# gradientpm/gvpm

Measured on AMD Instinct MI355X. Metric: photon gather+shift evaluations per second (G-BRE 3D), higher is better.
Workload: dtype f32; 1 GPU; BASELINE configs[1]: S-cbox + homogeneous medium, G-BRE 3D kernel, 512x512 frame, 1000000 photons/iter, 227 SPPM iters, initialScaleVolume 1.0; technique=bre3d, scene=cbox, photons_per_iter=1000000

## Files before the change

gvpm_amd/csrc/context.h:

```cpp
#pragma once
#include <dlfcn.h>
#include <hip/hip_runtime.h>
#include <rccl/rccl.h>

#include <cmath>
#include <cstdio>
#include <cstdlib>
#include <cstring>
#include <algorithm>
#include <chrono>
#include <string>
#include <vector>

#include "device_types.h"
#include "scene_bvh.h"

namespace gvpm {
hipError_t sortPairsU32(SortTemp &tmp, const uint32_t *kIn, uint32_t *kOut, const uint32_t *vIn, uint32_t *vOut,
                        uint32_t n, int endBit, hipStream_t s);
void launch_bounds(const float *pos, uint32_t n, float *partial, int nblocks, float *out6, float *hostOut,
                   hipStream_t s, const uint32_t *word = nullptr, uint32_t *wordOut = nullptr);
hipError_t reserveScanTemp(SortTemp &tmp, uint32_t n);
void launch_bundle_fit(const gvpm_camera_ray *rays, uint32_t nsets, int pass, const Grid &g, double *out, hipStream_t s);
void launch_export_u32(const uint32_t *a, const uint32_t *b, const uint32_t *c, const uint32_t *d, const uint32_t *e, uint32_t *hostOut,
// ... 19 lines not shown
void launch_tile_start(const uint32_t *start, uint32_t ntiles, uint32_t shift, uint32_t *tileStart, hipStream_t s);
void launch_segment_start(const uint32_t *keys, uint32_t n, uint32_t nseg, uint32_t shift, uint32_t *start,
                          hipStream_t s);
void launch_beam_keys(const gvpm_camera_ray *rays, uint32_t nsets, int width, int tw, int th, uint32_t *keys,
                      uint32_t *vals, hipStream_t s);
void launch_plan_bre(const GatherArgs &a, int beamsPerWave, uint32_t ntiles, uint32_t target, uint4 *items,
                     uint32_t *itemCount, uint2 *itemOff, uint32_t *blockTotal, uint32_t itemCap, hipStream_t stream);
uint32_t eval_unit_pairs();
void launch_traverse_bre(const GatherArgs &a, int beamsPerWave, const uint4 *items, const uint2 *itemOff,
                         const uint32_t *itemCount, uint32_t *queueHead, uint32_t *pairs, uint32_t *pairCnt,
                         uint32_t nwaves, bool persistent, hipStream_t stream, uint2 *units = nullptr, uint32_t *unitCtl = nullptr,
                         uint32_t unitCap = 0);
void launch_apply_host_shifts_beams(const GatherArgs &a, const gvpm_host_shift *results, uint32_t n, hipStream_t s);
void launch_evaluate_primal(const GatherArgs &a, int beamsPerWave, const uint4 *items, const uint2 *itemOff,
                            const uint32_t *itemCount, uint32_t *queueHead, const uint32_t *pairs, const uint32_t *pairCnt,
                            uint32_t nwaves, hipStream_t stream);
void launch_evaluate_bre(const GatherArgs &a, int beamsPerWave, bool fullVis, const uint4 *items, const uint2 *itemOff,
                         const uint32_t *itemCount, uint32_t *queueHead, const uint32_t *pairs, const uint32_t *pairCnt,
                         uint32_t nwaves, bool persistent, hipStream_t stream, const uint2 *units = nullptr,
                         const uint32_t *unitCtl = nullptr, uint32_t unitCap = 0);
uint32_t plan_items_capacity(uint32_t nsets, uint32_t ntiles, int beamsPerWave);
void launch_build_chain(ChainArgs c, const GatherArgs &a, const gvpm_photon_soa &raw, int beamsPerWave, uint32_t target, uint4 *items,
                        uint2 *itemOff, uint32_t itemCap, float dmax, const NearGrid &ng, uint32_t extCap, uint32_t *origIdx,
                        uint32_t *hostOut, bool initBuckets, hipStream_t s, uint32_t pairCapBlocks = 0xFFFFFFFFu, uint32_t unitCap = 0,
                        uint32_t unitPairs = 1, bool fullVis = false);
struct PoissonGraphCache {
  hipGraph_t graph = nullptr;
  hipGraphExec_t exec = nullptr;
  void *scratch = nullptr;
  int W = 0, H = 0, cgMax = 0;
  float alpha = 0.f;
};
void poisson_graph_release(PoissonGraphCache &c);
hipError_t poisson_solve_device(const gvpm_poisson_params &prm, int W, int H, const float *dx, const float *dy,
                                const float *tp, const float *direct, float *out, void *scratch,
                                PoissonGraphCache &cache, hipStream_t s);
size_t poisson_scratch_bytes(int W, int H);
void launch_finalize(float *accum, const float *iter, size_t n, int it, uint64_t nbPaths, hipStream_t s);
void launch_scale(const float *in, float *out, size_t n, float scale, hipStream_t s);
void launch_film(const float *acc, const float *emission, int w, int h, int it, int reusePrimal, float invDiv,
                 float *thr, float *dx, float *dy, hipStream_t s);
void launch_gather_vpm(const GatherArgs &a, bool fullVis, bool primal, hipStream_t stream);
void launch_vpm_find(const GatherArgs &a, const VpmSplit &sp, hipStream_t stream);
void launch_vpm_redo(const GatherArgs &a, const VpmSplit &sp, bool fullVis, uint32_t nwaves, hipStream_t stream);
void launch_vpm_eval(const GatherArgs &a, const VpmSplit &sp, bool fullVis, uint32_t wavesPerShard, hipStream_t stream);
void launch_vpm_finish(float *accum, float *iter, float *scaleVol, float *nVol, float *mvol, size_t n, float alpha,
                       uint32_t *maxScaleBits, hipStream_t stream);
void launch_accumulate(float *accum, float *iter, size_t n, uint32_t *zeroWord, hipStream_t stream);
// ... 127 lines not shown
  }
  void release() {
    hot.release(); cold.release(); overflowCtr.release(); origIdx.release(); cellStart.release(); cellCount.release(); cellSub.release(); sat.release();
    beamCount.release(); beamStart.release(); keysA.release(); keysB.release();
    valsA.release(); valsB.release(); boundsPartial.release(); bounds6.release(); bKeysA.release(); bKeysB.release();
    bValsA.release(); setPerm.release(); tileStart.release(); items.release(); itemOff.release(); planBoxes.release(); queueCtl.release();
    if (sortTmp.d) (void)hipFree(sortTmp.d);
    sortTmp.d = nullptr;
    sortTmp.bytes = 0;
    pairs.release(); pairCnt.release(); nearExt.release(); chainBuckets.release(); units.release(); notes.release(); notesCount.release();
    if (lastUse) (void)hipEventDestroy(lastUse);
    if (traversed) (void)hipEventDestroy(traversed);
    lastUse = traversed = nullptr;
  }
};

struct gvpm_context {
  int device = 0;
  hipStream_t stream = nullptr;
  hipStream_t streamB = nullptr;
  hipStream_t bstream = nullptr;
  hipStream_t streamC = nullptr;
  hipStream_t streamA2 = nullptr;
  bool evalAlt = false;
  int evalToggle = 0;
  hipEvent_t exactDone = nullptr;
  bool exactDoneValid = false;
  hipStream_t lastEvalStream = nullptr;
  bool travStream = true;
  BuildSet sets[3];
  BuildSet *bs = &sets[0];
  int setIdx = 0;
  bool travOnBuild = true;
  bool beamsExact = false;
  bool bundleEnabled = false;
  bool bundleFromEnv = false;
  bool bundleAuto = false;
  int bundleState = 0, bundleViolations = 0;
  int lastGridMode = 0;
  uint32_t lastGridCells = 0;
  float bundleDiv = 2.f;
  Grid bundleGrid{};
  bool buildChain = true;
  DevBuf<uint32_t> chainCtl;
  bool planBoxHandOff = true;
  bool beamsFreeCone = true;
// ... 209 lines not shown
```

gvpm_amd/csrc/gather_bre.hip:

```cpp
#include <hip/hip_runtime.h>

#include <cstdlib>
#include <type_traits>

#include "device_types.h"
#include "shift_device.h"
#include "tile_walk.h"
#include "vec.h"

namespace gvpm {

struct HitGeom {
  double disk, distSqr;
};

__device__ __forceinline__ HitGeom hitGeom(f3 pf, f3 of, f3 df) {
#pragma clang fp contract(off)
  const double px = pf.x, py = pf.y, pz = pf.z;
  const double ox = of.x, oy = of.y, oz = of.z;
  const double dx = df.x, dy = df.y, dz = df.z;
  const double cx = px - ox, cy = py - oy, cz = pz - oz;
  HitGeom g;
  g.disk = cx * dx + cy * dy + cz * dz;
  const double qx = ox + dx * g.disk, qy = oy + dy * g.disk, qz = oz + dz * g.disk;
// ... 400 lines not shown
  sf = sflux * ws;
  wb = bc * w;
}

template <int B, typename LDS> __device__ __forceinline__ void flushAcc(LDS &s, Acc27 &acc, uint32_t beam) {
#pragma unroll
  for (int k = 0; k < 27; ++k) {
    atomicAdd(&s.acc[k][beam], (double)(acc.v[k]));
    acc.v[k] = 0.f;
  }
}

__device__ __forceinline__ void waveLdsSync() {
  __builtin_amdgcn_fence(__ATOMIC_RELEASE, "wavefront");
  __builtin_amdgcn_wave_barrier();
  __builtin_amdgcn_fence(__ATOMIC_ACQUIRE, "wavefront");
}

#ifndef GVPM_TRAV_WPB
#define GVPM_TRAV_WPB 1
#endif
constexpr int TRAV_WPB = GVPM_TRAV_WPB;
#ifndef GVPM_TRAV_MINW
#define GVPM_TRAV_MINW 5
#endif
#ifndef GVPM_TRAV_OWN_MINW
#define GVPM_TRAV_OWN_MINW 4
#endif
#ifndef GVPM_EVAL_UNIT
#define GVPM_EVAL_UNIT 1280
#endif
#ifndef GVPM_EVAL_UNIT_SMALL
#define GVPM_EVAL_UNIT_SMALL 256
#endif
constexpr uint32_t EVAL_UNIT = GVPM_EVAL_UNIT, EVAL_UNIT_SMALL = GVPM_EVAL_UNIT_SMALL;
struct alignas(16) TravLds {
  float x[STAGE], y[STAGE], z[STAGE];
  uint32_t bits[STAGE];
  uint32_t stageIdx[STAGE];
  float4 cyl[3];
};
typedef float v2f __attribute__((ext_vector_type(2)));

template <int B, bool OWN_WALK>
__global__ __launch_bounds__(64 * TRAV_WPB) __attribute__((amdgpu_waves_per_eu(OWN_WALK ? GVPM_TRAV_OWN_MINW : GVPM_TRAV_MINW))) void traverse_bre_kernel(GatherArgs a, const uint4 *__restrict__ items,
                                                          const uint2 *__restrict__ itemOff,
                                                          const uint32_t *__restrict__ itemCount, uint32_t *queueHead,
// ... 202 lines not shown
                total += t;
              }
              if (B == 16) {
                const uint32_t t = (uint32_t)__shfl_xor((int)c, 16, 64);
                const uint32_t pairSum = c + t;
                const uint32_t t2 = (uint32_t)__shfl_xor((int)pairSum, 32, 64);
                before = ((lane & 16) ? t : 0u) + ((lane & 32) ? t2 : 0u);
                total = pairSum + t2;
              }
              uint32_t off = mine + before;
              while (cm) {
                const uint32_t u = (uint32_t)__ffs(cm) - 1u;
                cm &= cm - 1u;
                if (off < cap) outBase[outOff + off] = s.stageIdx[j0 + u];
                else nOver++;
                ++off;
              }
              mine += total;
            }
          }
        }
      }
    }
    if (sub == 0) pairCnt[(size_t)it * B + b] = (uint32_t)b < nb ? min(mine, cap) : 0u;
    if (units) {
      uint32_t tot = (sub == 0 && (uint32_t)b < nb) ? min(mine, cap) : 0u;
#pragma unroll
      for (int o = 32; o > 0; o >>= 1) tot += (uint32_t)__shfl_xor((int)tot, o, 64);
      tot = (uint32_t)__builtin_amdgcn_readfirstlane((int)tot);
      if (tot) {
        const uint32_t parts = (tot + EVAL_UNIT - 1u) / EVAL_UNIT;
        const uint32_t cls = (tot + parts - 1u) / parts > EVAL_UNIT_SMALL ? 0u : 1u;
        uint32_t slot = 0;
        if (lane == 0) slot = atomicAdd(&unitCtl[cls], parts);
        slot = (uint32_t)__builtin_amdgcn_readfirstlane((int)slot);
        for (uint32_t pp = (uint32_t)lane; pp < parts; pp += 64u) {
          if (slot + pp < unitCap) units[(size_t)cls * unitCap + slot + pp] = make_uint2(it, pp | (parts << 16));
          else nOver++;
        }
      }
    }
    nCand += tested * nb;
  }
  {
#pragma unroll
    for (int o = 32; o > 0; o >>= 1) nOver += (uint32_t)__shfl_xor((int)nOver, o, 64);
    if (lane == 0 && (nCand | nOver)) {
      unsigned long long *row = statRow(a);
      atomicAdd(&row[1], nCand);
      if (nOver) atomicAdd(&row[7], (unsigned long long)nOver);
    }
  }
}

#ifndef GVPM_EVAL_MINW
#define GVPM_EVAL_MINW 3
#endif
#ifndef GVPM_EVAL_ATTR
#define GVPM_EVAL_ATTR
#endif
// ... 567 lines not shown
```

gvpm_amd/csrc/gather_drivers.hip:

```cpp
#include "context.h"

float currentRadius(const gvpm_context *h) {
  return h->cfg.bsphere_radius * h->globalScaleVolume * 0.01f;
}

static int ilog2ceil(uint32_t v) {
  int b = 0;
  while ((1ull << b) < v) ++b;
  return b;
}

struct ChainPrep {
  bool on = false;
  float dmax = 0.f;
  bool wantOrig = false;
  uint32_t *sub = nullptr;
  uint32_t nkeys = 0, tileShift = 0;
  int tw = 4, th = 4;
};
static void beamTiling(const gvpm_context *h, int beamsPerWave, int &tw, int &th, uint32_t &ntiles, int &tileShift) {
  tw = 8;
  th = 4;
  if (beamsPerWave == 64) th = 8;
  if (beamsPerWave == 16) tw = 4;
// ... 658 lines not shown
    c.width = h->cfg.width;
    c.tw = cp.tw;
    c.th = cp.th;
    c.tileShift = cp.tileShift;
    c.ntiles = h->bs->ntiles;
    c.bKeys = h->bs->bKeysA.p;
    c.bRank = h->bs->bValsA.p;
    c.setPerm = h->bs->setPerm.p;
    c.tileStart = h->bs->tileStart.p;
    c.blockSum = reinterpret_cast<uint32_t *>(h->bs->sortTmp.d);
    c.ctl = h->chainCtl.p;
    c.queueCtl = h->bs->queueCtl.p;
    c.overflowCtr = h->bs->overflowCtr.p;
    c.nearExt = h->bs->nearExt.p;
    c.sat = h->bs->sat.p;
    h->boundsPending = h->haveCachedBounds;
    const bool optimistic = h->optimistic && h->pipeline && attempt == 0 && !primal && h->persistentEval && h->lastItems > 0 &&
                            h->bs->pairs.cap >= 128u && h->bs->pairCnt.cap >= (size_t)itemCap * h->beamsPerWave &&
                            (!h->evalUnits || h->bs->units.cap >= 2u);
    const bool fullVisOpt = !h->cfg.visibility_as_written || prevOverflow;
    const bool refuse = optimistic && h->optRefuseEvery > 0 && (++h->optSteps % h->optRefuseEvery) == 0;
    launch_build_chain(c, a, h->rawDev, h->beamsPerWave, h->planTarget, h->bs->items.p, h->bs->itemOff.p, itemCap, cp.dmax, h->nearGrid,
                       (uint32_t)std::min<size_t>(h->bs->nearExt.cap, 0xFFFFFF00u), cp.wantOrig ? h->bs->origIdx.p : nullptr, h->pinCtl,
                       !h->bs->bucketsInit, h->bstream,
                       optimistic ? (refuse ? 0u : (uint32_t)std::min<size_t>((h->bs->pairs.cap - 64u) / 64u, 0xFFFFFFF0u)) : 0xFFFFFFFFu,
                       optimistic && h->evalUnits ? (uint32_t)std::min<size_t>(h->bs->units.cap / 2u, 0x3FFFFFFFu) : 0u, eval_unit_pairs(),
                       fullVisOpt);
    h->bs->bucketsInit = true;
    chainRan = true;
    if (optimistic) {
      HIP_TRY(h, hipEventRecord(evBuild->second, h->bstream));
      const uint32_t guess = std::min<uint32_t>(itemCap, h->lastItems + h->lastItems / 8u + 256u);
      rc = queueGather(0u, guess, true, fullVisOpt);
      if (rc != GVPM_OK) {
        h->bstream = h->stream;
        return rc;
      }
      queued = true;
    }
  } else {
    HIP_TRY(h, hipMemsetAsync(h->bs->queueCtl.p, 0, 8 * sizeof(uint32_t), h->bstream));
    launch_plan_bre(a, h->beamsPerWave, h->bs->ntiles, h->planTarget, h->bs->items.p, h->bs->queueCtl.p, h->bs->itemOff.p,
                    h->bs->queueCtl.p + 3, itemCap, h->bstream);
    launch_export_u32(h->bs->queueCtl.p + 3, rebuilt ? h->bs->overflowCtr.p : nullptr, rebuilt ? h->bs->nearExt.p : nullptr,
                      h->bs->queueCtl.p, h->bs->queueCtl.p + 4, h->pinCtl, h->bstream);
  }
  if (!queued) HIP_TRY(h, hipEventRecord(evBuild->second, h->bstream));
  lap("plan");
  HIP_TRY(h, hipStreamSynchronize(h->bstream));
  lap("syncB");
  blocks = h->pinCtl[0];
  nItems = h->pinCtl[3];
  if (queued && h->pinCtl[5] != 0u) {
    if (getenv("GVPM_TRACE_PLAN")) fprintf(stderr, "[plan] optimistic step refused by the build (status %u): queued again\n", h->pinCtl[5]);
    HIP_TRY(h, hipStreamSynchronize(h->stream));
    if (h->pipeline && h->travStream) HIP_TRY(h, hipStreamSynchronize(h->streamC));
    HIP_TRY(h, hipMemsetAsync(h->bs->queueCtl.p + 1, 0, 2 * sizeof(uint32_t), h->bstream));
    HIP_TRY(h, hipMemsetAsync(h->bs->queueCtl.p + 5, 0, 3 * sizeof(uint32_t), h->bstream));
    HIP_TRY(h, hipStreamSynchronize(h->bstream));
    queued = false;
    h->optRefused++;
  }
  if (a.grid.mode == 1 && h->pinCtl[4] != 0u && attempt == 0) {
    h->bundleState = ++h->bundleViolations > 3 ? -1 : 0;
    h->photonsDirty = true;
    h->boundsPending = false;
    force3D = true;
    continue;
  }
  break;
  }
  h->lastGridMode = a.grid.mode;
  h->lastGridCells = a.grid.ncells;
  if (nItems > itemCap) {
    h->bstream = h->stream;
    return fail(h, GVPM_ERR_STATE, "G-BRE planner produced more work items than its bound");
  }
  if (getenv("GVPM_TRACE_PLAN")) {
    uint32_t q[4] = {0, 0, 0, 0};
// ... 704 lines not shown
```

gvpm_amd/csrc/grid_build.hip:

```cpp
#include <hip/hip_runtime.h>
#include <hipcub/hipcub.hpp>

#include "bundle_grid.h"
#include "device_types.h"
#include "shift_device.h"
#include "tile_walk.h"
#include "vec.h"

namespace gvpm {

__global__ __launch_bounds__(256) void bounds_kernel(const float *__restrict__ pos, uint32_t n, float *partial) {
  __shared__ float red[6][4];
  float mn[3] = {INFINITY, INFINITY, INFINITY}, mx[3] = {-INFINITY, -INFINITY, -INFINITY};
  for (uint32_t i = blockIdx.x * blockDim.x + threadIdx.x; i < n; i += gridDim.x * blockDim.x) {
#pragma unroll
    for (int c = 0; c < 3; ++c) {
      const float v = pos[3 * (size_t)i + c];
      mn[c] = fminf(mn[c], v);
      mx[c] = fmaxf(mx[c], v);
    }
  }
  const int wave = threadIdx.x / 64, lane = threadIdx.x % 64;
#pragma unroll
  for (int c = 0; c < 3; ++c) {
// ... 1112 lines not shown
  const uint32_t base = starts[c.beamOff];
  if (b < nSatBlocks + nBeamBlocks) {
    const uint32_t i = (b - nSatBlocks) * 256u + threadIdx.x;
    if (i < c.nsets) {
      const size_t k = (size_t)c.beamOff + c.bKeys[i];
      c.setPerm[starts[k] - base + (atomicSub(&c.counts[k], 1u) - 1u)] = i;
    }
    return;
  }
  const uint32_t t = (b - nSatBlocks - nBeamBlocks) * 256u + threadIdx.x;
  if (t <= c.ntiles) c.tileStart[t] = starts[(size_t)c.beamOff + ((size_t)t << c.tileShift)] - base;
}

struct TailArgs {
  uint32_t ntiles, target, itemCap, nPlan;
  uint4 *items;
  uint2 *itemOff;
  uint32_t *itemCount, *blockTotal;
  RawPhotons raw;
  const uint32_t *keys, *rank, *cellStart, *sub;
  uint32_t *counts;
  uint32_t *subCount;
  uint32_t n, ncells, extCap;
  uint32_t every;
  float dmax;
  NearGrid ng;
  uint32_t *nearExt, *overflow, *origIdx;
  float4 *hot, *cold;
  uint32_t *ctl;
  const uint32_t *bundleFlag;
  uint32_t *hostOut;
  uint32_t pairCapBlocks;
  uint32_t unitCap, unitPairs;
  uint32_t fullVis;
  uint32_t planGroups;
};
constexpr uint32_t TAIL_PLAN_STAGE = 128;
template <int B> constexpr size_t tailLdsBytes() {
  constexpr size_t pl = sizeof(PlanLds<B, TAIL_PLAN_STAGE>) > sizeof(PlanLdsQ<B, TAIL_PLAN_STAGE>) ? sizeof(PlanLds<B, TAIL_PLAN_STAGE>)
                                                                                                  : sizeof(PlanLdsQ<B, TAIL_PLAN_STAGE>);
  return pl > sizeof(ReorderLds) ? pl : sizeof(ReorderLds);
}
#ifndef GVPM_TAIL_WPE
#define GVPM_TAIL_WPE 6
#endif
template <int B, int MODE> __global__ __launch_bounds__(64) __attribute__((amdgpu_waves_per_eu(GVPM_TAIL_WPE, GVPM_TAIL_WPE))) void chain_tail_kernel(GatherArgs a, TailArgs t) {
  __shared__ __attribute__((aligned(16))) unsigned char ldsRaw[tailLdsBytes<B>()];
  const uint32_t b = blockIdx.x, pslot = b / t.every;
  if (b % t.every == 0u && pslot < t.nPlan) {
    if (a.grid.mode != 1 && t.planGroups)
      planBodyQ<B, TAIL_PLAN_STAGE>(a, t.ntiles, t.target, t.items, t.itemCount, t.itemOff, t.blockTotal, t.itemCap, pslot, t.nPlan,
                                    *reinterpret_cast<PlanLdsQ<B, TAIL_PLAN_STAGE> *>(ldsRaw));
    else
      planBody<B, TAIL_PLAN_STAGE>(a, t.ntiles, t.target, t.items, t.itemCount, t.itemOff, t.blockTotal, t.itemCap, pslot, t.nPlan,
                                   *reinterpret_cast<PlanLds<B, TAIL_PLAN_STAGE> *>(ldsRaw));
  }
  else
    reorderBody<MODE>(t.raw, t.keys, t.rank, t.cellStart, t.n, a.cfg, a.bvh, a.tri4, a.ntri, t.dmax, t.ng, t.nearExt, t.extCap, t.hot,
                      t.cold, t.overflow, t.origIdx, t.sub, t.ncells, b - min(t.nPlan, (b + t.every - 1u) / t.every), t.counts,
                      t.subCount, *reinterpret_cast<ReorderLds *>(ldsRaw));
  if (!lastBlockArrives(t.ctl, blockIdx.x, gridDim.x)) return;
  if (threadIdx.x == 0) {
    t.hostOut[0] = coherentRead(t.blockTotal);
    t.hostOut[1] = coherentRead(t.overflow);
    t.hostOut[2] = coherentRead(t.nearExt);
    t.hostOut[3] = coherentRead(t.itemCount);
    t.hostOut[4] = t.bundleFlag ? coherentRead(const_cast<uint32_t *>(t.bundleFlag)) : 0u;
    uint32_t bad = 0u;
    if (t.pairCapBlocks != 0xFFFFFFFFu) {
      const uint32_t blocks = t.hostOut[0], nIt = t.hostOut[3];
      if (blocks > t.pairCapBlocks) bad |= 1u;
      if (nIt > t.itemCap) bad |= 2u;
      if (t.unitCap && (unsigned long long)blocks * 64ull / t.unitPairs + nIt + 64ull > (unsigned long long)t.unitCap) bad |= 4u;
      if (t.hostOut[1] != 0u && !t.fullVis) bad |= 8u;
      if (t.hostOut[4] != 0u) bad |= 16u;
    }
    t.itemCount[7] = bad;
    t.hostOut[5] = bad;
    __threadfence_system();
  }
}

template <int B>
static void launchTail(int mode, uint32_t grid, hipStream_t s, const GatherArgs &a, const TailArgs &t) {
  if (mode == 0) hipLaunchKernelGGL((chain_tail_kernel<B, 0>), dim3(grid), dim3(64), 0, s, a, t);
  else if (mode == 2) hipLaunchKernelGGL((chain_tail_kernel<B, 2>), dim3(grid), dim3(64), 0, s, a, t);
  else hipLaunchKernelGGL((chain_tail_kernel<B, 1>), dim3(grid), dim3(64), 0, s, a, t);
}

void launch_build_chain(ChainArgs c, const GatherArgs &a, const gvpm_photon_soa &raw, int beamsPerWave, uint32_t target, uint4 *items,
                        uint2 *itemOff, uint32_t itemCap, float dmax, const NearGrid &ng, uint32_t extCap, uint32_t *origIdx,
                        uint32_t *hostOut, bool initBuckets, hipStream_t s, uint32_t pairCapBlocks, uint32_t unitCap, uint32_t unitPairs,
                        bool fullVis) {
  c.nPhBlocks = (c.n + 255u) / 256u;
  c.nBeamBlocks = (c.nsets + 255u) / 256u;
  if (initBuckets) hipLaunchKernelGGL(chain_init_buckets_kernel, dim3(1), dim3(768), 0, s, c.buckets);
  hipLaunchKernelGGL(chain_count_kernel, dim3(c.nPhBlocks + c.nBeamBlocks), dim3(256), 0, s, c);
  if (c.g.mode == 1)
    hipLaunchKernelGGL(chain_stripes_kernel, dim3((c.g.ncells + 255) / 256), dim3(256), 0, s, c.sub, c.sub + (size_t)CELL_STRIPES * c.g.ncells,
                       c.g.ncells, c.counts);
  const uint32_t nScan = (c.scanLen + SCAN_TILE - 1) / SCAN_TILE;
  hipLaunchKernelGGL(chain_scan_reduce_kernel, dim3(nScan), dim3(SCAN_BLOCK), 0, s, c);
  hipLaunchKernelGGL(chain_scan_down_kernel, dim3(nScan), dim3(SCAN_BLOCK), 0, s, c);
  const uint32_t nx1 = c.g.dim[0] + 1, ny1 = c.g.dim[1] + 1;
  const uint32_t nSat = (nx1 * (uint32_t)c.g.dim[2] + 255u) / 256u, nTile = (c.ntiles + 1u + 255u) / 256u;
  hipLaunchKernelGGL(chain_mid_kernel, dim3(nSat + c.nBeamBlocks + nTile), dim3(256), 0, s, c, nSat, c.nBeamBlocks);
  hipLaunchKernelGGL(sat_z_kernel, dim3((nx1 * ny1 + 255) / 256), dim3(256), 0, s, c.g, c.sat);
  TailArgs t{};
  t.ntiles = c.ntiles;
  t.target = target;
  t.itemCap = itemCap;
  t.planGroups = getenv("GVPM_PLAN_GROUPS") ? (atoi(getenv("GVPM_PLAN_GROUPS")) != 0) : 1u;
  {
    const uint32_t per = (t.planGroups && c.g.mode != 1) ? (uint32_t)(64 / (beamsPerWave > 0 ? beamsPerWave : 16)) : 1u;
    const uint32_t want = (c.ntiles + per - 1u) / per;
    t.nPlan = want < 4093u ? std::max(1u, want) : 4093u;
// ... 9 lines not shown
  t.rank = c.rank;
  t.cellStart = c.starts;
  t.sub = c.g.mode == 1 ? c.sub + (size_t)CELL_STRIPES * c.g.ncells : nullptr;
  t.subCount = c.g.mode == 1 ? c.sub : nullptr;
  t.counts = c.g.mode == 1 ? nullptr : c.counts;
  t.n = c.n;
  t.ncells = c.g.ncells;
  t.extCap = extCap;
  t.dmax = dmax;
  t.ng = ng;
  t.nearExt = c.nearExt;
  t.overflow = c.overflowCtr;
  t.origIdx = origIdx;
  t.hot = const_cast<float4 *>(a.hot);
  t.cold = const_cast<float4 *>(a.cold);
  t.ctl = c.ctl + 65;
  t.bundleFlag = a.bundleFlag;
  t.hostOut = hostOut;
  t.pairCapBlocks = pairCapBlocks;
  t.unitCap = unitCap;
  t.unitPairs = unitPairs ? unitPairs : 1u;
  t.fullVis = fullVis ? 1u : 0u;
  const int mode = a.ntri <= 64u ? 0 : (ng.start ? 2 : 1);
  const uint32_t grid = t.nPlan + (c.n + 63u) / 64u;
  t.every = std::max(1u, grid / std::max(1u, t.nPlan));
  switch (beamsPerWave) {
    case 64: launchTail<64>(mode, grid, s, a, t); break;
    case 32: launchTail<32>(mode, grid, s, a, t); break;
    default: launchTail<16>(mode, grid, s, a, t); break;
  }
}

}
```

gvpm_amd/csrc/gvpm_api.hip:

```cpp
#include "context.h"

RcclApi g_rccl;

static const char *validateParams(const gvpm_params *p) {
  if (p->abi_version != GVPM_ABI_VERSION) return "abi_version mismatch";
  if (p->width <= 0 || p->height <= 0 || p->width > 65535 || p->height > 65535) return "bad film size";
  if (p->vol_technique < GVPM_VOL_BRE2D || p->vol_technique > GVPM_VOL_PLANE0D) return "unknown vol_technique";
  const bool use3D = p->vol_technique == GVPM_DISTANCE || p->vol_technique == GVPM_VOL_BRE3D ||
                     (p->vol_technique >= GVPM_BEAM_BEAM_3D_NAIVE && p->vol_technique <= GVPM_BEAM_BEAM_3D_OPTIMIZED);
  if (p->use_shift_null && !use3D && p->vol_technique != GVPM_BEAM_BEAM_1D)
    return "Not possible to shift null without using 3D kernel";
  if (p->max_depth <= 1 && p->max_depth != -1 && p->max_depth != 0) return "Maximum depth must be set to \"2\" or higher!";
  if (!(p->bsphere_radius > 0.f)) return "bsphere_radius must be positive";
  if (!(p->epsilon > 0.f) || !(p->shadow_epsilon > 0.f)) return "epsilon / shadow_epsilon must be positive";
  if (!std::isfinite(p->alpha) || !(p->alpha > 0.f) || p->alpha > 1.f) return "alpha must be in (0, 1]";
  if (p->vol_technique == GVPM_VOL_PLANE0D && p->min_depth < 2) return "Impossible to use plane with minDepth smaller than 2";
  if (!p->no_medium_shift) return "noMediumShift=false is not supported (shiftPhotonMedium is SAssert(false))";
  return nullptr;
}

extern "C" {

int gvpm_abi_version(void) { return GVPM_ABI_VERSION; }

// ... 5 lines not shown
  if (validateParams(params)) {
    const char *m = validateParams(params);
    return (strstr(m, "shift null") || strstr(m, "noMediumShift")) ? GVPM_ERR_UNSUPPORTED : GVPM_ERR_INVALID_ARG;
  }
  int ndev = 0;
  if (hipGetDeviceCount(&ndev) != hipSuccess || ndev <= 0 || device < 0 || device >= ndev) return GVPM_ERR_NO_DEVICE;
  if (hipSetDevice(device) != hipSuccess) return GVPM_ERR_NO_DEVICE;
  gvpm_context *h = new gvpm_context();
  h->device = device;
  h->cfg = *params;
  int prA = 0, prB = 1, prC = -1;
  {
    int least = 0, greatest = 0;
    if (hipDeviceGetStreamPriorityRange(&least, &greatest) == hipSuccess) {
      prB = std::min(prB, least);
      prC = std::max(prC, greatest);
    }
  }
  if (const char *e = getenv("GVPM_STREAM_PRIORITIES")) (void)sscanf(e, "%d,%d,%d", &prA, &prB, &prC);
  if (hipStreamCreateWithPriority(&h->stream, hipStreamNonBlocking, prA) != hipSuccess ||
      hipStreamCreateWithPriority(&h->streamB, hipStreamNonBlocking, prB) != hipSuccess ||
      hipStreamCreateWithPriority(&h->streamC, hipStreamNonBlocking, prC) != hipSuccess ||
      hipStreamCreateWithPriority(&h->streamA2, hipStreamNonBlocking, prA) != hipSuccess ||
      hipEventCreateWithFlags(&h->sets[0].lastUse, hipEventDisableTiming) != hipSuccess ||
      hipEventCreateWithFlags(&h->sets[1].lastUse, hipEventDisableTiming) != hipSuccess ||
      hipEventCreateWithFlags(&h->sets[2].lastUse, hipEventDisableTiming) != hipSuccess ||
      hipEventCreateWithFlags(&h->sets[0].traversed, hipEventDisableTiming) != hipSuccess ||
      hipEventCreateWithFlags(&h->sets[1].traversed, hipEventDisableTiming) != hipSuccess ||
      hipEventCreateWithFlags(&h->sets[2].traversed, hipEventDisableTiming) != hipSuccess) {
    gvpm_destroy(h);
    return GVPM_ERR_HIP;
  }
  if (hipStreamCreateWithFlags(&h->copyStream, hipStreamNonBlocking) != hipSuccess) {
    gvpm_destroy(h);
    return GVPM_ERR_HIP;
  }
  for (int k = 0; k < 3; ++k)
    if (hipEventCreateWithFlags(&h->phSlot[k].copied, hipEventDisableTiming) != hipSuccess ||
        hipEventCreateWithFlags(&h->phSlot[k].consumed, hipEventDisableTiming) != hipSuccess ||
        hipEventCreateWithFlags(&h->phSlot[k].consumedB, hipEventDisableTiming) != hipSuccess ||
        hipEventCreateWithFlags(&h->raySlot[k].copied, hipEventDisableTiming) != hipSuccess ||
        hipEventCreateWithFlags(&h->raySlot[k].freed, hipEventDisableTiming) != hipSuccess) {
      gvpm_destroy(h);
      return GVPM_ERR_HIP;
    }
  h->bstream = h->stream;
// ... 32 lines not shown
  if (const char *e = getenv("GVPM_TRAV_WAVES_PER_CU")) {
    int v = atoi(e);
    if (v >= 1 && v <= 32) h->nwavesTrav = h->ncu * (uint32_t)v;
  }
  {
    if (h->nwavesTrav > GVPM_STAT_ROWS) h->nwavesTrav = GVPM_STAT_ROWS;
    if (h->nwaves > GVPM_STAT_ROWS) h->nwaves = GVPM_STAT_ROWS;
  }
  if (const char *e = getenv("GVPM_PIPELINE")) h->pipeline = atoi(e) != 0;
  if (!h->pipeline && !getenv("GVPM_WAVES_PER_CU") && h->ncu) h->nwaves = std::min<uint32_t>(h->ncu * 12u, GVPM_STAT_ROWS);
  if (const char *e = getenv("GVPM_PERSISTENT")) h->persistentEval = (atoi(e) & 1) != 0, h->persistentTrav = (atoi(e) & 2) != 0;
  if (const char *e = getenv("GVPM_TRAV_ON_BUILD")) h->travOnBuild = atoi(e) != 0;
  if (const char *e = getenv("GVPM_NEAR_GRID")) h->useNearGrid = atoi(e) != 0;
  if (const char *e = getenv("GVPM_TRAV_STREAM")) h->travStream = atoi(e) != 0;
  if (const char *e = getenv("GVPM_BEAMS_FP64")) h->beamsExact = atoi(e) != 0;
  if (const char *e = getenv("GVPM_BEAMS_FREE_CONE")) h->beamsFreeCone = atoi(e) != 0;
  if (const char *e = getenv("GVPM_PLAN_BOXES")) h->planBoxHandOff = atoi(e) != 0;
  if (const char *e = getenv("GVPM_BUILD_CHAIN")) h->buildChain = atoi(e) != 0;
  if (const char *e = getenv("GVPM_EVAL_UNITS")) h->evalUnits = atoi(e) != 0;
  if (const char *e = getenv("GVPM_OPTIMISTIC")) h->optimistic = atoi(e) != 0;
  if (const char *e = getenv("GVPM_OPTIMISTIC_REFUSE")) h->optRefuseEvery = (uint32_t)std::max(0, atoi(e));
  if (const char *e = getenv("GVPM_CLIP_GRID")) h->clipGrid = atoi(e) != 0;
  if (const char *e = getenv("GVPM_EVAL_ALT")) h->evalAlt = atoi(e) != 0;
  if (const char *e = getenv("GVPM_VPM_ORDER")) h->vpmNoOrder = atoi(e) == 0;
  if (const char *e = getenv("GVPM_VPM_SPLIT")) h->vpmSplit = atoi(e) != 0;
  if (const char *e = getenv("GVPM_VPM_PIPELINE")) h->vpmPipeline = atoi(e) != 0;
  if (const char *e = getenv("GVPM_VPM_POOL")) h->vpmPoolPerBatch = (uint32_t)std::max(0, atoi(e));
  if (const char *e = getenv("GVPM_VPM_EVAL_WAVES")) h->vpmEvalWaves = (uint32_t)std::max(64, atoi(e));
  if (const char *e = getenv("GVPM_VPM_REDO_WAVES")) h->vpmRedoWaves = (uint32_t)std::max(1, atoi(e));
  if (const char *e = getenv("GVPM_BEAMS_SPLIT")) h->beamsSplit = atoi(e) != 0;
  if (const char *e = getenv("GVPM_BUNDLE_AUTO")) h->bundleAuto = atoi(e) != 0;
  if (const char *e = getenv("GVPM_BUNDLE")) {
    h->bundleEnabled = atoi(e) != 0;
    h->bundleFromEnv = true;
  }
  if (const char *e = getenv("GVPM_BUNDLE_DIV")) {
    const float v = (float)atof(e);
    if (v >= 0.25f && v <= 16.f) h->bundleDiv = v;
  }
  if (const char *e = getenv("GVPM_BEAM_PAIRS_INIT")) {
    const long long v = atoll(e);
    if (v >= 64 && v <= ((long long)1 << 31)) h->beamPairsInit = (size_t)v;
  }
  if (const char *e = getenv("GVPM_BEAM_ITEMS_INIT")) {
    const long long v = atoll(e);
    if (v >= 1 && v <= ((long long)1 << 30)) h->beamItemsInit = (uint32_t)v;
// ... 20 lines not shown
  }
  *out = h;
  int rc = gvpm_reset(h);
  if (rc != GVPM_OK) {
    gvpm_destroy(h);
    *out = nullptr;
  }
  return rc;
}

int gvpm_destroy(gvpm_context *h) {
  if (!h) return GVPM_ERR_INVALID_ARG;
  (void)hipSetDevice(h->device);
  if (h->stream) (void)hipStreamSynchronize(h->stream);
  if (h->comm && g_rccl.commDestroy) g_rccl.commDestroy(h->comm);
  for (auto &v : h->events)
    for (auto &e : v) {
      (void)hipEventDestroy(e.first);
      (void)hipEventDestroy(e.second);
    }
  if (h->streamB) (void)hipStreamSynchronize(h->streamB);
  if (h->streamC) (void)hipStreamSynchronize(h->streamC);
  if (h->streamA2) (void)hipStreamSynchronize(h->streamA2);
  for (BuildSet &b : h->sets) b.release();
  h->tri4.release(); h->bvh.release();
  for (auto &ps : h->phSlot) {
    ps.raw.release();
    ps.packed.release();
    if (ps.unpacked) (void)hipEventDestroy(ps.unpacked);
    if (ps.copied) (void)hipEventDestroy(ps.copied);
    if (ps.consumed) (void)hipEventDestroy(ps.consumed);
    if (ps.consumedB) (void)hipEventDestroy(ps.consumedB);
  }
  for (auto &rs : h->raySlot) {
    rs.rays.release();
    rs.packed.release();
    if (rs.unpacked) (void)hipEventDestroy(rs.unpacked);
    if (rs.copied) (void)hipEventDestroy(rs.copied);
    if (rs.freed) (void)hipEventDestroy(rs.freed);
  }
  if (h->copyStream) (void)hipStreamDestroy(h->copyStream);
  h->materials.release();
  h->reqHost.release(); h->reqCtx.release(); h->reqCount.release(); h->reqResults.release();
  h->endNOwned.release(); h->subCounts.release(); h->subOffsets.release();
  h->beamCtl.release(); h->beamAux.release(); h->beamClear.release();
  h->nearGridStart.release(); h->nearGridTris.release(); h->nearGridCount.release();
  h->w1Owned.release(); h->len1Owned.release(); h->planeTest.release(); h->beamPairs.release(); h->subFlags.release(); h->shiftExtent.release();
  h->blockKeyA.release(); h->blockKeyB.release(); h->blockValA.release(); h->blockValB.release();
  h->samplesOwned.release(); h->scaleVol.release(); h->nVol.release(); h->mvol.release(); h->maxScaleBits.release();
  poisson_graph_release(h->poissonGraph);
  h->accumTmp.release();
  h->chainCtl.release();
  h->poissonScratch.release(); h->poissonIO.release();
  h->accum.release(); h->accumAll.release(); h->iter.release(); h->filmOut.release(); h->emission.release(); h->stats.release();
  h->exPay.release(); h->exPayCount.release(); h->exOvf.release(); h->exOvfCount.release(); h->exTotals.release();
  if (h->pinB6) (void)hipHostFree(h->pinB6);
  if (h->pinExact) (void)hipHostFree(h->pinExact);
  if (h->pinBeams) (void)hipHostFree(h->pinBeams);
  h->splitId.release(); h->splitMeta.release(); h->splitBlkCnt.release(); h->splitCtl.release(); h->splitK.release();
  h->splitU.release(); h->splitRuns.release();
  if (h->stream) (void)hipStreamDestroy(h->stream);
  if (h->streamB) (void)hipStreamDestroy(h->streamB);
  if (h->streamC) (void)hipStreamDestroy(h->streamC);
  if (h->streamA2) (void)hipStreamDestroy(h->streamA2);
  if (h->exactDone) (void)hipEventDestroy(h->exactDone);
  h->vpmPairs.release(); h->vpmChunkMeta.release(); h->vpmCtl.release(); h->vpmStatus.release(); h->vpmRedo.release(); h->vpmState.release();
  if (h->vpmFound) (void)hipEventDestroy(h->vpmFound);
  if (h->vpmRedone) (void)hipEventDestroy(h->vpmRedone);
  delete h;
  return GVPM_OK;
}

int gvpm_reset(gvpm_context *h) {
  CHECK_H(h);
  {
    const int rcj = joinEvalStreams(h);
    if (rcj != GVPM_OK) return rcj;
  }
  h->reqOutstanding = false;
  h->reqBeams = false;
  if (h->reqCount.p) HIP_TRY(h, hipMemsetAsync(h->reqCount.p, 0, 8, h->stream));
  h->vpmOrderN = 0;
  h->vpmLaunches = 0;
  HIP_TRY(h, hipMemsetAsync(h->exPayCount.p, 0, 4 * sizeof(uint32_t), h->stream));
  HIP_TRY(h, hipMemsetAsync(h->exOvfCount.p, 0, 4 * sizeof(uint32_t), h->stream));
  h->exSince = 0;
  HIP_TRY(h, hipMemsetAsync(h->exTotals.p, 0, 32 * sizeof(unsigned long long), h->stream));
// ... 398 lines not shown
```

Baseline: 6419 Mevals/s.

## Split chain tail into concurrent plan and scatter kernels on separate streams

Replaces the fused chain tail kernel, which interleaved plan blocks and reorder blocks in one grid, with two kernels. The scatter kernel runs on a new stream forked and joined with events, so it can overlap the plan kernel. Each kernel gets its own waves-per-EU bound and LDS size, and whichever block arrives last across both grids writes the host export. The change also raises the traversal min-waves bound and hints scalar-register row pointers for the pairCnt and unit stores. Risks are the extra event and launch overhead, and correctness of the shared last-block counter across two grids running concurrently.

```diff
diff --git a/gvpm_amd/csrc/context.h b/gvpm_amd/csrc/context.h
--- a/gvpm_amd/csrc/context.h
+++ b/gvpm_amd/csrc/context.h
@@ -65,8 +65,8 @@
 uint32_t plan_items_capacity(uint32_t nsets, uint32_t ntiles, int beamsPerWave);
 void launch_build_chain(ChainArgs c, const GatherArgs &a, const gvpm_photon_soa &raw, int beamsPerWave, uint32_t target, uint4 *items,
                         uint2 *itemOff, uint32_t itemCap, float dmax, const NearGrid &ng, uint32_t extCap, uint32_t *origIdx,
-                        uint32_t *hostOut, bool initBuckets, hipStream_t s, uint32_t pairCapBlocks = 0xFFFFFFFFu, uint32_t unitCap = 0,
-                        uint32_t unitPairs = 1, bool fullVis = false);
+                        uint32_t *hostOut, bool initBuckets, hipStream_t s, hipStream_t scatterStream, hipEvent_t fork, hipEvent_t join,
+                        uint32_t pairCapBlocks = 0xFFFFFFFFu, uint32_t unitCap = 0, uint32_t unitPairs = 1, bool fullVis = false);
 struct PoissonGraphCache {
   hipGraph_t graph = nullptr;
   hipGraphExec_t exec = nullptr;
@@ -240,6 +240,9 @@
   hipStream_t bstream = nullptr;
   hipStream_t streamC = nullptr;
   hipStream_t streamA2 = nullptr;
+  hipStream_t streamB2 = nullptr;
+  hipEvent_t tailFork = nullptr, tailJoin = nullptr;
+  bool tailSplit = true;
   bool evalAlt = false;
   int evalToggle = 0;
   hipEvent_t exactDone = nullptr;
diff --git a/gvpm_amd/csrc/gather_bre.hip b/gvpm_amd/csrc/gather_bre.hip
--- a/gvpm_amd/csrc/gather_bre.hip
+++ b/gvpm_amd/csrc/gather_bre.hip
@@ -446,7 +446,7 @@
 #endif
 constexpr int TRAV_WPB = GVPM_TRAV_WPB;
 #ifndef GVPM_TRAV_MINW
-#define GVPM_TRAV_MINW 5
+#define GVPM_TRAV_MINW 6
 #endif
 #ifndef GVPM_TRAV_OWN_MINW
 #define GVPM_TRAV_OWN_MINW 4
@@ -695,7 +695,11 @@
         }
       }
     }
-    if (sub == 0) pairCnt[(size_t)it * B + b] = (uint32_t)b < nb ? min(mine, cap) : 0u;
+    {
+      uint32_t *cntRow = pairCnt + (size_t)it * B;
+      asm volatile("" : "+s"(cntRow));
+      if (sub == 0) cntRow[b] = (uint32_t)b < nb ? min(mine, cap) : 0u;
+    }
     if (units) {
       uint32_t tot = (sub == 0 && (uint32_t)b < nb) ? min(mine, cap) : 0u;
 #pragma unroll
@@ -707,8 +711,10 @@
         uint32_t slot = 0;
         if (lane == 0) slot = atomicAdd(&unitCtl[cls], parts);
         slot = (uint32_t)__builtin_amdgcn_readfirstlane((int)slot);
+        uint2 *unitRow = units + ((size_t)cls * unitCap + slot);
+        asm volatile("" : "+s"(unitRow));
         for (uint32_t pp = (uint32_t)lane; pp < parts; pp += 64u) {
-          if (slot + pp < unitCap) units[(size_t)cls * unitCap + slot + pp] = make_uint2(it, pp | (parts << 16));
+          if (slot + pp < unitCap) unitRow[pp] = make_uint2(it, pp | (parts << 16));
           else nOver++;
         }
       }
diff --git a/gvpm_amd/csrc/gather_drivers.hip b/gvpm_amd/csrc/gather_drivers.hip
--- a/gvpm_amd/csrc/gather_drivers.hip
+++ b/gvpm_amd/csrc/gather_drivers.hip
@@ -704,7 +704,7 @@
     const bool refuse = optimistic && h->optRefuseEvery > 0 && (++h->optSteps % h->optRefuseEvery) == 0;
     launch_build_chain(c, a, h->rawDev, h->beamsPerWave, h->planTarget, h->bs->items.p, h->bs->itemOff.p, itemCap, cp.dmax, h->nearGrid,
                        (uint32_t)std::min<size_t>(h->bs->nearExt.cap, 0xFFFFFF00u), cp.wantOrig ? h->bs->origIdx.p : nullptr, h->pinCtl,
-                       !h->bs->bucketsInit, h->bstream,
+                       !h->bs->bucketsInit, h->bstream, h->tailSplit ? h->streamB2 : nullptr, h->tailFork, h->tailJoin,
                        optimistic ? (refuse ? 0u : (uint32_t)std::min<size_t>((h->bs->pairs.cap - 64u) / 64u, 0xFFFFFFF0u)) : 0xFFFFFFFFu,
                        optimistic && h->evalUnits ? (uint32_t)std::min<size_t>(h->bs->units.cap / 2u, 0x3FFFFFFFu) : 0u, eval_unit_pairs(),
                        fullVisOpt);
@@ -737,6 +737,7 @@
     if (getenv("GVPM_TRACE_PLAN")) fprintf(stderr, "[plan] optimistic step refused by the build (status %u): queued again\n", h->pinCtl[5]);
     HIP_TRY(h, hipStreamSynchronize(h->stream));
     if (h->pipeline && h->travStream) HIP_TRY(h, hipStreamSynchronize(h->streamC));
+    if (h->streamB2) HIP_TRY(h, hipStreamSynchronize(h->streamB2));
     HIP_TRY(h, hipMemsetAsync(h->bs->queueCtl.p + 1, 0, 2 * sizeof(uint32_t), h->bstream));
     HIP_TRY(h, hipMemsetAsync(h->bs->queueCtl.p + 5, 0, 3 * sizeof(uint32_t), h->bstream));
     HIP_TRY(h, hipStreamSynchronize(h->bstream));
diff --git a/gvpm_amd/csrc/grid_build.hip b/gvpm_amd/csrc/grid_build.hip
--- a/gvpm_amd/csrc/grid_build.hip
+++ b/gvpm_amd/csrc/grid_build.hip
@@ -1158,7 +1158,7 @@
   uint32_t *counts;
   uint32_t *subCount;
   uint32_t n, ncells, extCap;
-  uint32_t every;
+  uint32_t nScatter;
   float dmax;
   NearGrid ng;
   uint32_t *nearExt, *overflow, *origIdx;
@@ -1172,62 +1172,60 @@
   uint32_t planGroups;
 };
 constexpr uint32_t TAIL_PLAN_STAGE = 128;
-template <int B> constexpr size_t tailLdsBytes() {
-  constexpr size_t pl = sizeof(PlanLds<B, TAIL_PLAN_STAGE>) > sizeof(PlanLdsQ<B, TAIL_PLAN_STAGE>) ? sizeof(PlanLds<B, TAIL_PLAN_STAGE>)
-                                                                                                  : sizeof(PlanLdsQ<B, TAIL_PLAN_STAGE>);
-  return pl > sizeof(ReorderLds) ? pl : sizeof(ReorderLds);
-}
+template <int B> constexpr size_t planLdsBytes() {
+  return sizeof(PlanLds<B, TAIL_PLAN_STAGE>) > sizeof(PlanLdsQ<B, TAIL_PLAN_STAGE>) ? sizeof(PlanLds<B, TAIL_PLAN_STAGE>)
+                                                                                    : sizeof(PlanLdsQ<B, TAIL_PLAN_STAGE>);
+}
+#ifndef GVPM_SCATTER_WPE
+#define GVPM_SCATTER_WPE 8
+#endif
 #ifndef GVPM_TAIL_WPE
 #define GVPM_TAIL_WPE 6
 #endif
-template <int B, int MODE> __global__ __launch_bounds__(64) __attribute__((amdgpu_waves_per_eu(GVPM_TAIL_WPE, GVPM_TAIL_WPE))) void chain_tail_kernel(GatherArgs a, TailArgs t) {
-  __shared__ __attribute__((aligned(16))) unsigned char ldsRaw[tailLdsBytes<B>()];
-  const uint32_t b = blockIdx.x, pslot = b / t.every;
-  if (b % t.every == 0u && pslot < t.nPlan) {
-    if (a.grid.mode != 1 && t.planGroups)
-      planBodyQ<B, TAIL_PLAN_STAGE>(a, t.ntiles, t.target, t.items, t.itemCount, t.itemOff, t.blockTotal, t.itemCap, pslot, t.nPlan,
-                                    *reinterpret_cast<PlanLdsQ<B, TAIL_PLAN_STAGE> *>(ldsRaw));
-    else
-      planBody<B, TAIL_PLAN_STAGE>(a, t.ntiles, t.target, t.items, t.itemCount, t.itemOff, t.blockTotal, t.itemCap, pslot, t.nPlan,
-                                   *reinterpret_cast<PlanLds<B, TAIL_PLAN_STAGE> *>(ldsRaw));
-  }
+#ifndef GVPM_PLAN_WPE
+#define GVPM_PLAN_WPE 6
+#endif
+__device__ __forceinline__ void tailExport(const TailArgs &t) {
+  if (threadIdx.x != 0) return;
+  t.hostOut[0] = coherentRead(t.blockTotal);
+  t.hostOut[1] = coherentRead(t.overflow);
+  t.hostOut[2] = coherentRead(t.nearExt);
+  t.hostOut[3] = coherentRead(t.itemCount);
+  t.hostOut[4] = t.bundleFlag ? coherentRead(const_cast<uint32_t *>(t.bundleFlag)) : 0u;
+  uint32_t bad = 0u;
+  if (t.pairCapBlocks != 0xFFFFFFFFu) {
+    const uint32_t blocks = t.hostOut[0], nIt = t.hostOut[3];
+    if (blocks > t.pairCapBlocks) bad |= 1u;
+    if (nIt > t.itemCap) bad |= 2u;
+    if (t.unitCap && (unsigned long long)blocks * 64ull / t.unitPairs + nIt + 64ull > (unsigned long long)t.unitCap) bad |= 4u;
+    if (t.hostOut[1] != 0u && !t.fullVis) bad |= 8u;
+    if (t.hostOut[4] != 0u) bad |= 16u;
+  }
+  t.itemCount[7] = bad;
+  t.hostOut[5] = bad;
+  __threadfence_system();
+}
+template <int B> __global__ __launch_bounds__(64) __attribute__((amdgpu_waves_per_eu(GVPM_PLAN_WPE, GVPM_PLAN_WPE))) void chain_plan_kernel(GatherArgs a, TailArgs t) {
+  __shared__ __attribute__((aligned(16))) unsigned char ldsRaw[planLdsBytes<B>()];
+  if (a.grid.mode != 1 && t.planGroups)
+    planBodyQ<B, TAIL_PLAN_STAGE>(a, t.ntiles, t.target, t.items, t.itemCount, t.itemOff, t.blockTotal, t.itemCap, blockIdx.x, t.nPlan,
+                                  *reinterpret_cast<PlanLdsQ<B, TAIL_PLAN_STAGE> *>(ldsRaw));
   else
-    reorderBody<MODE>(t.raw, t.keys, t.rank, t.cellStart, t.n, a.cfg, a.bvh, a.tri4, a.ntri, t.dmax, t.ng, t.nearExt, t.extCap, t.hot,
-                      t.cold, t.overflow, t.origIdx, t.sub, t.ncells, b - min(t.nPlan, (b + t.every - 1u) / t.every), t.counts,
-                      t.subCount, *reinterpret_cast<ReorderLds *>(ldsRaw));
-  if (!lastBlockArrives(t.ctl, blockIdx.x, gridDim.x)) return;
-  if (threadIdx.x == 0) {
-    t.hostOut[0] = coherentRead(t.blockTotal);
-    t.hostOut[1] = coherentRead(t.overflow);
-    t.hostOut[2] = coherentRead(t.nearExt);
-    t.hostOut[3] = coherentRead(t.itemCount);
-    t.hostOut[4] = t.bundleFlag ? coherentRead(const_cast<uint32_t *>(t.bundleFlag)) : 0u;
-    uint32_t bad = 0u;
-    if (t.pairCapBlocks != 0xFFFFFFFFu) {
-      const uint32_t blocks = t.hostOut[0], nIt = t.hostOut[3];
-      if (blocks > t.pairCapBlocks) bad |= 1u;
-      if (nIt > t.itemCap) bad |= 2u;
-      if (t.unitCap && (unsigned long long)blocks * 64ull / t.unitPairs + nIt + 64ull > (unsigned long long)t.unitCap) bad |= 4u;
-      if (t.hostOut[1] != 0u && !t.fullVis) bad |= 8u;
-      if (t.hostOut[4] != 0u) bad |= 16u;
-    }
-    t.itemCount[7] = bad;
-    t.hostOut[5] = bad;
-    __threadfence_system();
-  }
-}
-
-template <int B>
-static void launchTail(int mode, uint32_t grid, hipStream_t s, const GatherArgs &a, const TailArgs &t) {
-  if (mode == 0) hipLaunchKernelGGL((chain_tail_kernel<B, 0>), dim3(grid), dim3(64), 0, s, a, t);
-  else if (mode == 2) hipLaunchKernelGGL((chain_tail_kernel<B, 2>), dim3(grid), dim3(64), 0, s, a, t);
-  else hipLaunchKernelGGL((chain_tail_kernel<B, 1>), dim3(grid), dim3(64), 0, s, a, t);
+    planBody<B, TAIL_PLAN_STAGE>(a, t.ntiles, t.target, t.items, t.itemCount, t.itemOff, t.blockTotal, t.itemCap, blockIdx.x, t.nPlan,
+                                 *reinterpret_cast<PlanLds<B, TAIL_PLAN_STAGE> *>(ldsRaw));
+  if (lastBlockArrives(t.ctl, blockIdx.x, t.nPlan + t.nScatter)) tailExport(t);
+}
+template <int MODE> __global__ __launch_bounds__(64) __attribute__((amdgpu_waves_per_eu(MODE == 0 ? GVPM_SCATTER_WPE : GVPM_TAIL_WPE, MODE == 0 ? GVPM_SCATTER_WPE : GVPM_TAIL_WPE))) void chain_scatter_kernel(GatherArgs a, TailArgs t) {
+  __shared__ ReorderLds lds;
+  reorderBody<MODE>(t.raw, t.keys, t.rank, t.cellStart, t.n, a.cfg, a.bvh, a.tri4, a.ntri, t.dmax, t.ng, t.nearExt, t.extCap, t.hot,
+                    t.cold, t.overflow, t.origIdx, t.sub, t.ncells, blockIdx.x, t.counts, t.subCount, lds);
+  if (lastBlockArrives(t.ctl, t.nPlan + blockIdx.x, t.nPlan + t.nScatter)) tailExport(t);
 }
 
 void launch_build_chain(ChainArgs c, const GatherArgs &a, const gvpm_photon_soa &raw, int beamsPerWave, uint32_t target, uint4 *items,
                         uint2 *itemOff, uint32_t itemCap, float dmax, const NearGrid &ng, uint32_t extCap, uint32_t *origIdx,
-                        uint32_t *hostOut, bool initBuckets, hipStream_t s, uint32_t pairCapBlocks, uint32_t unitCap, uint32_t unitPairs,
-                        bool fullVis) {
+                        uint32_t *hostOut, bool initBuckets, hipStream_t s, hipStream_t scatterStream, hipEvent_t fork, hipEvent_t join,
+                        uint32_t pairCapBlocks, uint32_t unitCap, uint32_t unitPairs, bool fullVis) {
   c.nPhBlocks = (c.n + 255u) / 256u;
   c.nBeamBlocks = (c.nsets + 255u) / 256u;
   if (initBuckets) hipLaunchKernelGGL(chain_init_buckets_kernel, dim3(1), dim3(768), 0, s, c.buckets);
@@ -1283,13 +1281,26 @@
   t.unitPairs = unitPairs ? unitPairs : 1u;
   t.fullVis = fullVis ? 1u : 0u;
   const int mode = a.ntri <= 64u ? 0 : (ng.start ? 2 : 1);
-  const uint32_t grid = t.nPlan + (c.n + 63u) / 64u;
-  t.every = std::max(1u, grid / std::max(1u, t.nPlan));
+  t.nScatter = (c.n + 63u) / 64u;
+  hipStream_t ss = scatterStream && fork && join ? scatterStream : s;
+  if (ss != s) {
+    (void)hipEventRecord(fork, s);
+    (void)hipStreamWaitEvent(ss, fork, 0);
+  }
+  if (t.nScatter) {
+    if (mode == 0) hipLaunchKernelGGL(chain_scatter_kernel<0>, dim3(t.nScatter), dim3(64), 0, ss, a, t);
+    else if (mode == 2) hipLaunchKernelGGL(chain_scatter_kernel<2>, dim3(t.nScatter), dim3(64), 0, ss, a, t);
+    else hipLaunchKernelGGL(chain_scatter_kernel<1>, dim3(t.nScatter), dim3(64), 0, ss, a, t);
+  }
   switch (beamsPerWave) {
-    case 64: launchTail<64>(mode, grid, s, a, t); break;
-    case 32: launchTail<32>(mode, grid, s, a, t); break;
-    default: launchTail<16>(mode, grid, s, a, t); break;
-  }
-}
-
-}
+    case 64: hipLaunchKernelGGL(chain_plan_kernel<64>, dim3(t.nPlan), dim3(64), 0, s, a, t); break;
+    case 32: hipLaunchKernelGGL(chain_plan_kernel<32>, dim3(t.nPlan), dim3(64), 0, s, a, t); break;
+    default: hipLaunchKernelGGL(chain_plan_kernel<16>, dim3(t.nPlan), dim3(64), 0, s, a, t); break;
+  }
+  if (ss != s) {
+    (void)hipEventRecord(join, ss);
+    (void)hipStreamWaitEvent(s, join, 0);
+  }
+}
+
+}
diff --git a/gvpm_amd/csrc/gvpm_api.hip b/gvpm_amd/csrc/gvpm_api.hip
--- a/gvpm_amd/csrc/gvpm_api.hip
+++ b/gvpm_amd/csrc/gvpm_api.hip
@@ -51,6 +51,9 @@
       hipStreamCreateWithPriority(&h->streamB, hipStreamNonBlocking, prB) != hipSuccess ||
       hipStreamCreateWithPriority(&h->streamC, hipStreamNonBlocking, prC) != hipSuccess ||
       hipStreamCreateWithPriority(&h->streamA2, hipStreamNonBlocking, prA) != hipSuccess ||
+      hipStreamCreateWithPriority(&h->streamB2, hipStreamNonBlocking, prB) != hipSuccess ||
+      hipEventCreateWithFlags(&h->tailFork, hipEventDisableTiming) != hipSuccess ||
+      hipEventCreateWithFlags(&h->tailJoin, hipEventDisableTiming) != hipSuccess ||
       hipEventCreateWithFlags(&h->sets[0].lastUse, hipEventDisableTiming) != hipSuccess ||
       hipEventCreateWithFlags(&h->sets[1].lastUse, hipEventDisableTiming) != hipSuccess ||
       hipEventCreateWithFlags(&h->sets[2].lastUse, hipEventDisableTiming) != hipSuccess ||
@@ -129,6 +132,7 @@
   if (const char *e = getenv("GVPM_OPTIMISTIC_REFUSE")) h->optRefuseEvery = (uint32_t)std::max(0, atoi(e));
   if (const char *e = getenv("GVPM_CLIP_GRID")) h->clipGrid = atoi(e) != 0;
   if (const char *e = getenv("GVPM_EVAL_ALT")) h->evalAlt = atoi(e) != 0;
+  if (const char *e = getenv("GVPM_TAIL_SPLIT")) h->tailSplit = atoi(e) != 0;
   if (const char *e = getenv("GVPM_VPM_ORDER")) h->vpmNoOrder = atoi(e) == 0;
   if (const char *e = getenv("GVPM_VPM_SPLIT")) h->vpmSplit = atoi(e) != 0;
   if (const char *e = getenv("GVPM_VPM_PIPELINE")) h->vpmPipeline = atoi(e) != 0;
@@ -195,6 +199,7 @@
   if (h->streamB) (void)hipStreamSynchronize(h->streamB);
   if (h->streamC) (void)hipStreamSynchronize(h->streamC);
   if (h->streamA2) (void)hipStreamSynchronize(h->streamA2);
+  if (h->streamB2) (void)hipStreamSynchronize(h->streamB2);
   for (BuildSet &b : h->sets) b.release();
   h->tri4.release(); h->bvh.release();
   for (auto &ps : h->phSlot) {
@@ -236,6 +241,9 @@
   if (h->streamB) (void)hipStreamDestroy(h->streamB);
   if (h->streamC) (void)hipStreamDestroy(h->streamC);
   if (h->streamA2) (void)hipStreamDestroy(h->streamA2);
+  if (h->streamB2) (void)hipStreamDestroy(h->streamB2);
+  if (h->tailFork) (void)hipEventDestroy(h->tailFork);
+  if (h->tailJoin) (void)hipEventDestroy(h->tailJoin);
   if (h->exactDone) (void)hipEventDestroy(h->exactDone);
   h->vpmPairs.release(); h->vpmChunkMeta.release(); h->vpmCtl.release(); h->vpmStatus.release(); h->vpmRedo.release(); h->vpmState.release();
   if (h->vpmFound) (void)hipEventDestroy(h->vpmFound);
```

Result: slower. 5944 Mevals/s (median of 2 runs) (-7.4%).
